# numz/ComfyUI-SeedVR2_VideoUpscaler

Measured on AMD Instinct MI355X. Metric: upscaled frames/sec (720p->4K, SeedVR2-3B), higher is better.
Workload: dtype bf16; 1 GPU; cfg3: SeedVR2-3B 32-frame 720p->4K clip (padded to 33 = 4n+1 for encode + DiT, 32 decoded), VAE tiled 1024/128; vae_tiled=True, parallelism=dp1, weights=random-init SeedVR2-3B + video_vae_v3 architecture (seeded)

## Files before the change

### comfyui-seedvr2_videoupscaler_amd/csrc/svr_conv_halo2.hip

```cpp
#include "svr_common.h"
#include "../../include/seedvr2_hip.h"
#include <type_traits>

namespace svr {

constexpr int CG_TX = 32, CG_HX = CG_TX + 2;
constexpr int CG_BUNIT = 128 * 64;
constexpr int CG_NB = 8;
constexpr int CG_D = 4;
static_assert(CG_D < CG_NB, "ring slot of unit k + D must not hold a unit still being read");

template <int TY, int MODE> struct cg_geom {
    static constexpr int MTW = MODE == 3 ? 8 : 4;
    static constexpr int NT = MODE == 3 ? 256 : TY * 32;
    static constexpr int HY = TY + 2;
    static constexpr int ROWS = CG_HX * HY;
    static constexpr int ACHUNKS = ROWS * 4;
    static constexpr int PIECES = (ACHUNKS + NT - 1) / NT;
    static constexpr int ABUF = MODE == 3 ? PIECES * NT * 16 : ROWS * 64;
    static constexpr int BOFF = 2 * ABUF;
    static constexpr int EP_ROWS = MODE ? 4 : 8;
    static constexpr int EP_BYTES = EP_ROWS * 32 * 528;
    static constexpr int THIN_PITCH = 272;
    static constexpr int MAIN = MODE == 2 ? TY * 32 * THIN_PITCH : (MODE == 1 || MODE == 3 ? BOFF : BOFF + CG_NB * CG_BUNIT);
    static constexpr int LDS = MAIN > EP_BYTES ? MAIN : EP_BYTES;
    static_assert(MODE == 3 || PIECES <= 7, "the next halo must have landed before interval 8");
};

template <int N> SVR_DEVICE void cg_wait_vmcnt() { asm volatile("s_waitcnt vmcnt(%0)" ::"n"(N) : "memory"); }
template <int OFF> SVR_DEVICE void cg_rd2(bf16x8 (&r)[2], unsigned a0) {
    asm volatile("ds_read_b128 %0, %2 offset:%3\n\tds_read_b128 %1, %2 offset:%4"
                 : "=&v"(r[0]), "=&v"(r[1]) : "v"(a0), "n"(OFF), "n"(OFF + 1024) : "memory");
}
SVR_DEVICE void cg_mm4(f32x4 (&c)[2][2], const bf16x8 (&w)[2], const bf16x8 (&r)[2]) {
    c[0][0] = __builtin_amdgcn_mfma_f32_16x16x32_bf16(w[0], r[0], c[0][0], 0, 0, 0);
    c[0][1] = __builtin_amdgcn_mfma_f32_16x16x32_bf16(w[1], r[0], c[0][1], 0, 0, 0);
    c[1][0] = __builtin_amdgcn_mfma_f32_16x16x32_bf16(w[0], r[1], c[1][0], 0, 0, 0);
    c[1][1] = __builtin_amdgcn_mfma_f32_16x16x32_bf16(w[1], r[1], c[1][1], 0, 0, 0);
}
SVR_DEVICE void cg_mm4_inplace(f32x4 (&c)[2][2], const bf16x8 (&w)[2], const bf16x8 (&r)[2]) {
    asm volatile("v_mfma_f32_16x16x32_bf16 %0, %1, %2, %0" : "+v"(c[0][0]) : "v"(w[0]), "v"(r[0]));
    asm volatile("v_mfma_f32_16x16x32_bf16 %0, %1, %2, %0" : "+v"(c[0][1]) : "v"(w[1]), "v"(r[0]));
    asm volatile("v_mfma_f32_16x16x32_bf16 %0, %1, %2, %0" : "+v"(c[1][0]) : "v"(w[0]), "v"(r[1]));
    asm volatile("v_mfma_f32_16x16x32_bf16 %0, %1, %2, %0" : "+v"(c[1][1]) : "v"(w[1]), "v"(r[1]));
}
template <int N> SVR_DEVICE void cg_wait_rows(bf16x8 (&a)[2]) {
    asm volatile("s_waitcnt lgkmcnt(%2)" : "+v"(a[0]), "+v"(a[1]) : "n"(N));
    __builtin_amdgcn_sched_barrier(0);
}
template <int N> SVR_DEVICE void cg_wait_rows(bf16x8 (&a)[2], bf16x8 (&b)[2]) {
    asm volatile("s_waitcnt lgkmcnt(%4)" : "+v"(a[0]), "+v"(a[1]), "+v"(b[0]), "+v"(b[1]) : "n"(N));
    __builtin_amdgcn_sched_barrier(0);
}
template <int N> SVR_DEVICE void cg_wait_rows(bf16x8 (&a)[2], bf16x8 (&b)[2], bf16x8 (&c)[2], bf16x8 (&d)[2], bf16x8 (&e)[2],
                                              bf16x8 (&f)[2], bf16x8 (&g)[2], bf16x8 (&h)[2]) {
    asm volatile("s_waitcnt lgkmcnt(%16)"
                 : "+v"(a[0]), "+v"(a[1]), "+v"(b[0]), "+v"(b[1]), "+v"(c[0]), "+v"(c[1]), "+v"(d[0]), "+v"(d[1]),
                   "+v"(e[0]), "+v"(e[1]), "+v"(f[0]), "+v"(f[1]), "+v"(g[0]), "+v"(g[1]), "+v"(h[0]), "+v"(h[1]) : "n"(N));
    __builtin_amdgcn_sched_barrier(0);
}
template <int N> SVR_DEVICE void cg_wait_w(bf16x8 (&w)[2][2]) {
    asm volatile("s_waitcnt vmcnt(%4)" : "+v"(w[0][0]), "+v"(w[0][1]), "+v"(w[1][0]), "+v"(w[1][1]) : "n"(N));
    __builtin_amdgcn_sched_barrier(0);
}

#ifdef SVR_ABLATIONS
__device__ unsigned long long g_conv_tl[4096][4];
__device__ unsigned long long g_conv_ep[4096][16];
#endif
template <int TY, int MODE, int DBG = 0>
__global__ __launch_bounds__((cg_geom<TY, MODE>::NT), (MODE == 3 ? 1 : 2)) void conv_halo2_kernel(const svr_gemm_args a, const int band_rows) {
#ifndef SVR_ABLATIONS
    static_assert(DBG == 0, "measurement variants (results invalid on purpose) exist only in -DSVR_ABLATIONS builds; the product library instantiates DBG = 0");
#endif
    typedef cg_geom<TY, MODE> G;
    constexpr bool WREG = MODE == 1 || MODE == 3, W8 = MODE == 3, THIN = MODE == 2;
    constexpr int CG_TY = TY, CG_ROWS = G::ROWS, CG_ABUF = G::ABUF, CG_ACHUNKS = G::ACHUNKS, CG_PIECES = G::PIECES,
                  CG_BOFF = G::BOFF, NT = G::NT;
    constexpr int MTW = G::MTW, NTW = 2;
    extern __shared__ __attribute__((aligned(16))) char smem[];

    const svr_conv_geom& g = a.conv;
    const int tid = threadIdx.x;
#ifdef SVR_ABLATIONS
    if constexpr ((DBG & 256) != 0) { if (tid == 0 && blockIdx.x < 4096) g_conv_tl[blockIdx.x][0] = __builtin_amdgcn_s_memtime(); }
#endif
    const int lane = tid & 63;
    const int wave = __builtin_amdgcn_readfirstlane(tid >> 6);
    const int grp = wave >> 2;
    const int wm = wave >> 1, wn = wave & 1;

    const int tiles_x = (g.W + CG_TX - 1) / CG_TX;
    const int tiles_y = (g.H + CG_TY - 1) / CG_TY;
    const int tiles_n = a.N / 128;
    int tl;
    {
        const int nwg = gridDim.x, bid = blockIdx.x;
        const int xcd = bid & 7, j = bid >> 3, q = nwg >> 3, r = nwg & 7;
        tl = (xcd < r ? xcd * (q + 1) : r * (q + 1) + (xcd - r) * q) + j;
    }
    const int tn = tl % tiles_n;
    int rr = tl / tiles_n;
    const int tx = rr % tiles_x; rr /= tiles_x;
    int ty, to;
    if (band_rows > 0 && band_rows < tiles_y) {
        const int per_band = band_rows * g.To;
        const int b = rr / per_band;
        const int rows_b = min(band_rows, tiles_y - b * band_rows);
        const int r2 = rr - b * per_band;
        to = r2 / rows_b;
        ty = b * band_rows + (r2 - to * rows_b);
    } else {
        ty = rr % tiles_y;
        to = rr / tiles_y;
    }
    const int y0 = ty * CG_TY, x0 = tx * CG_TX, n0 = tn * 128;

    const int cpk = THIN ? 1 : g.Cin / 32;
    const int nA = g.kt * cpk;
    const int P = nA * 9;
    const int64_t frame_bytes = (int64_t)g.H * g.W * g.Cin * 2;
    const int srow = tid >> 2, spos = tid & 3;
    const char* wbase = (const char*)a.W + (int64_t)(n0 + srow) * a.K * 2 + ((spos ^ ((srow >> 2) & 3)) * 16);
    uint32_t poff[CG_PIECES];
    uint32_t akeys = 0;
#pragma unroll
    for (int q = 0; q < CG_PIECES; ++q) {
        const int row = q * (NT / 4) + srow;
        const int hy = row / CG_HX, hx = row - hy * CG_HX;
        const int y = y0 - 1 + hy, x = x0 - 1 + hx;
        const bool ok = row < CG_ROWS && (unsigned)y < (unsigned)g.H && (unsigned)x < (unsigned)g.W;
        poff[q] = ok ? (uint32_t)(y * g.W + x) : 0xffffffffu;
        akeys |= (uint32_t)(spos ^ ((hx >> 2) & 3)) << (2 * q);
    }
    char* const wave_dst = smem + wave * 1024;

    auto frame_ptr = [&](int s) -> const char* {
        const int dt = s / cpk;
        const int c0 = (s - dt * cpk) * 32;
        int f = to + dt - g.pt;
        const char* basep = (const char*)a.A;
        if (f < 0) {
            if (g.halo != nullptr) { basep = (const char*)g.halo; f += g.halo_frames; }
            else f = 0;
        }
        return basep + (int64_t)f * frame_bytes + c0 * 2;
    };
    auto stage_a_piece = [&](auto qc, const char* fptr, int buf) {
        constexpr int Q = decltype(qc)::value;
        if (Q * NT + wave * 64 >= CG_ACHUNKS) return false;
        const int ck = (akeys >> (2 * Q)) & 3;
        const char* src = poff[Q] == 0xffffffffu ? (const char*)g.zeros
                                                 : fptr + ((int64_t)poff[Q] * g.Cin + ck * 8) * 2;
        if constexpr (!(DBG & 2))
            if (Q * NT + tid < CG_ACHUNKS) glds16(src, wave_dst + buf * CG_ABUF + Q * (NT * 16));
        return true;
    };
    auto stage_b = [&](int s, int tap, int slot) {
        const int dt = s / cpk;
        const int c0 = (s - dt * cpk) * 32;
        const int64_t koff = ((int64_t)(dt * 9 + tap) * g.Cin + c0) * 2;
        glds16(wbase + koff, wave_dst + CG_BOFF + slot * CG_BUNIT);
    };

    const int l15 = lane & 15, c4 = lane >> 4;
    int rd_a0[3], rd_b0;
#pragma unroll
    for (int dx = 0; dx < 3; ++dx)
        rd_a0[dx] = (wm * MTW * CG_HX + l15) * 64 + ((c4 ^ (((dx + l15) >> 2) & 3)) << 4);
    rd_b0 = CG_BOFF + (wn * 64 + l15) * 64 + ((c4 ^ ((l15 >> 2) & 3)) << 4);

    f32x4 acc[MTW][NTW][2][2];
#pragma unroll
    for (int y = 0; y < MTW; ++y)
#pragma unroll
        for (int z = 0; z < NTW; ++z)
#pragma unroll
            for (int e = 0; e < 16; ++e) acc[y][z][e >> 3][(e >> 2) & 1][e & 3] = 0.f;
    bf16x8 ar0[2], ar1[2], ar2[2], ar3[2], ar4[2], ar5[2], wf[NTW][2];
    bf16x8 ar6[2], ar7[2], ar8[2], ar9[2];

    auto reads = [&](auto jc, int s, int k) {
        constexpr int J = decltype(jc)::value;
        constexpr int DY = J % 3, DX = J / 3;
        int ra = rd_a0[DX] + (s & 1) * CG_ABUF;
        int rb = rd_b0 + (k & (CG_NB - 1)) * CG_BUNIT;
        asm volatile("" : "+v"(ra), "+v"(rb));
#pragma unroll
        for (int ks = 0; ks < 2; ++ks) {
            const char* pa = smem + ra + ks * 1024;
            const char* pb = smem + rb + ks * 1024;
            if constexpr (DY == 0) {
                ar0[ks] = *(const bf16x8*)(pa + (0 * CG_HX + DX) * 64);
                ar1[ks] = *(const bf16x8*)(pa + (1 * CG_HX + DX) * 64);
                ar2[ks] = *(const bf16x8*)(pa + (2 * CG_HX + DX) * 64);
                ar3[ks] = *(const bf16x8*)(pa + (3 * CG_HX + DX) * 64);
            } else if constexpr (DY == 1) {
                ar4[ks] = *(const bf16x8*)(pa + (4 * CG_HX + DX) * 64);
            } else {
                ar5[ks] = *(const bf16x8*)(pa + (5 * CG_HX + DX) * 64);
            }
#pragma unroll
            for (int nt = 0; nt < NTW; ++nt) wf[nt][ks] = *(const bf16x8*)(pb + nt * (32 * 64));
        }
    };
    auto mfma_core = [&](const bf16x8 (&r0)[2], const bf16x8 (&r1)[2], const bf16x8 (&r2)[2], const bf16x8 (&r3)[2]) {
        __builtin_amdgcn_s_setprio(1);
        cg_mm4(acc[0][0], wf[0], r0); cg_mm4(acc[0][1], wf[1], r0); cg_mm4(acc[1][0], wf[0], r1); cg_mm4(acc[1][1], wf[1], r1);
        cg_mm4(acc[2][0], wf[0], r2); cg_mm4(acc[2][1], wf[1], r2); cg_mm4(acc[3][0], wf[0], r3); cg_mm4(acc[3][1], wf[1], r3);
        __builtin_amdgcn_s_setprio(0);
    };
    auto mfmas = [&](auto jc) {
        constexpr int DY = decltype(jc)::value % 3;
        if constexpr (DY == 0) mfma_core(ar0, ar1, ar2, ar3);
        else if constexpr (DY == 1) mfma_core(ar1, ar2, ar3, ar4);
        else mfma_core(ar2, ar3, ar4, ar5);
    };

    if constexpr (THIN) {
        constexpr int TP = G::THIN_PITCH;
        static_assert(NT == 256, "one voxel per thread");
        const int taps = g.kt * 9;
        {
            const int y = y0 + (tid >> 5), x = x0 + (tid & 31);
            char* rowp = smem + tid * TP;
            const int64_t fpix = (int64_t)g.H * g.W;
            uint2 vv[32];
#pragma unroll
            for (int tap = 0; tap < 32; ++tap) {
                uint2 v = make_uint2(0u, 0u);
                if (tap < taps) {
                    const int dt = tap / 9, r = tap - dt * 9, dy = r / 3, dx = r - dy * 3;
                    const int ys = y + dy - 1, xs = x + dx - 1;
                    if ((unsigned)ys < (unsigned)g.H && (unsigned)xs < (unsigned)g.W) {
                        int f = to + dt - g.pt;
                        const char* basep = (const char*)a.A;
                        if (f < 0) {
                            if (g.halo != nullptr) { basep = (const char*)g.halo; f += g.halo_frames; }
                            else f = 0;
                        }
                        v = *(const uint2*)(basep + ((int64_t)f * fpix + (int64_t)ys * g.W + xs) * 8);
                    }
                }
                vv[tap] = v;
            }
#pragma unroll
            for (int tap = 0; tap < 32; tap += 2)
                *(uint4*)(rowp + tap * 8) = make_uint4(vv[tap].x, vv[tap].y, vv[tap + 1].x, vv[tap + 1].y);
        }
        __syncthreads();
        const int nks = (taps * 4 + 31) >> 5;
        const char* wrow0 = (const char*)a.W + ((int64_t)(n0 + wn * 64 + l15) * a.K + c4 * 8) * 2;
        const char* arow0 = smem + ((wm * MTW) * 32 + l15) * TP + c4 * 16;
#pragma unroll
        for (int ks = 0; ks < 4; ++ks) {
            if (ks < nks) {
                bf16x8 b[NTW][2];
#pragma unroll
                for (int q = 0; q < 2 * NTW; ++q) b[q >> 1][q & 1] = *(const bf16x8*)(wrow0 + (int64_t)(16 * q) * a.K * 2 + ks * 64);
#pragma unroll
                for (int mt = 0; mt < MTW; ++mt) {
                    bf16x8 av[2];
                    av[0] = *(const bf16x8*)(arow0 + mt * 32 * TP + ks * 64);
                    av[1] = *(const bf16x8*)(arow0 + (mt * 32 + 16) * TP + ks * 64);
                    cg_mm4(acc[mt][0], b[0], av);
                    cg_mm4(acc[mt][1], b[1], av);
                }
            }
        }
        __syncthreads();
    } else
    if constexpr (WREG) {
        const int64_t nstride = (int64_t)P * 2048;
        const char* wp0 = (const char*)a.W_frag + (int64_t)(n0 / 32 + wn * 2) * nstride;
        const char* wp1 = wp0 + nstride;
        const int voff = c4 * 512 + l15 * 16;
        bf16x8 w0[NTW][2], w1[NTW][2], w2[NTW][2];
        auto wload = [&](bf16x8 (&w)[NTW][2], int k) {
            if constexpr ((DBG & 32) != 0) k &= 3;
            auto uniform_ptr = [](const char* p) {
                const uint64_t u = (uint64_t)p;
                const uint32_t lo = __builtin_amdgcn_readfirstlane((uint32_t)u), hi = __builtin_amdgcn_readfirstlane((uint32_t)(u >> 32));
                return (const char*)(((uint64_t)hi << 32) | lo);
            };
            const char* p0 = uniform_ptr(wp0 + (int64_t)min(k, P - 1) * 2048);
            const char* p1 = uniform_ptr(wp1 + (int64_t)min(k, P - 1) * 2048);
            if constexpr ((DBG & 1) != 0 && W8) {
                if (k > 2) return;
            } else if constexpr (DBG & 1) {
                const bf16x8 z = {0, 0, 0, 0, 0, 0, 0, 0};
                w[0][0] = z; w[0][1] = z; w[1][0] = z; w[1][1] = z;
                return;
            }
            asm volatile("global_load_dwordx4 %0, %1, %2" : "=v"(w[0][0]) : "v"(voff), "s"(p0) : "memory");
            asm volatile("global_load_dwordx4 %0, %1, %2 offset:256" : "=v"(w[0][1]) : "v"(voff), "s"(p0) : "memory");
            asm volatile("global_load_dwordx4 %0, %1, %2" : "=v"(w[1][0]) : "v"(voff), "s"(p1) : "memory");
            asm volatile("global_load_dwordx4 %0, %1, %2 offset:256" : "=v"(w[1][1]) : "v"(voff), "s"(p1) : "memory");
        };
        auto reads_a = [&](auto jc, int s) {
            constexpr int J = decltype(jc)::value;
            constexpr int DY = J % 3, DX = J / 3;
            if constexpr ((DBG & 64) != 0) { if (s > 0) return; }
            int ra = rd_a0[DX] + (s & 1) * CG_ABUF;
            asm volatile("" : "+v"(ra));
#pragma unroll
            for (int ks = 0; ks < 2; ++ks) {
                const char* pa = smem + ra + ks * 1024;
                if constexpr (DY == 0) {
                    ar0[ks] = *(const bf16x8*)(pa + (0 * CG_HX + DX) * 64);
                    ar1[ks] = *(const bf16x8*)(pa + (1 * CG_HX + DX) * 64);
                    ar2[ks] = *(const bf16x8*)(pa + (2 * CG_HX + DX) * 64);
                    ar3[ks] = *(const bf16x8*)(pa + (3 * CG_HX + DX) * 64);
                } else if constexpr (DY == 1) {
                    ar4[ks] = *(const bf16x8*)(pa + (4 * CG_HX + DX) * 64);
                } else {
                    ar5[ks] = *(const bf16x8*)(pa + (5 * CG_HX + DX) * 64);
                }
            }
        };
        auto mfma_w = [&](const bf16x8 (&w)[NTW][2], const bf16x8 (&r0)[2], const bf16x8 (&r1)[2],
                          const bf16x8 (&r2)[2], const bf16x8 (&r3)[2]) {
            cg_mm4_inplace(acc[0][0], w[0], r0); cg_mm4_inplace(acc[0][1], w[1], r0);
            cg_mm4_inplace(acc[1][0], w[0], r1); cg_mm4_inplace(acc[1][1], w[1], r1);
            cg_mm4_inplace(acc[2][0], w[0], r2); cg_mm4_inplace(acc[2][1], w[1], r2);
            cg_mm4_inplace(acc[3][0], w[0], r3); cg_mm4_inplace(acc[3][1], w[1], r3);
        };
        if constexpr (W8) {
        const unsigned lds0 = (unsigned)(uintptr_t)(__attribute__((address_space(3))) char*)smem;
        unsigned fa[3];
#pragma unroll
        for (int dx = 0; dx < 3; ++dx) fa[dx] = lds0 + (unsigned)rd_a0[dx];
        auto stage_full = [&](auto qc, const char* fptr, int buf) {
            constexpr int Q = decltype(qc)::value;
            const int ck = (akeys >> (2 * Q)) & 3;
            const char* src = (poff[Q] == 0xffffffffu || fptr == nullptr) ? (const char*)g.zeros
                                                                          : fptr + ((int64_t)poff[Q] * g.Cin + ck * 8) * 2;
            glds16(src, wave_dst + buf * CG_ABUF + Q * (NT * 16));
        };
        static_assert(CG_PIECES == 10, "piece schedule below is written for ten pieces, two per interval 0..4");
        constexpr bool ABL_NO_DMA = (DBG & 16) != 0, ABL_NO_W = (DBG & 1) != 0, ABL_NO_RD = (DBG & 64) != 0;
#define SVR_RD(ROW, R, DXV, BUFOFF) do { if constexpr (!ABL_NO_RD) cg_rd2<((R) * CG_HX + (DXV)) * 64>(ROW, fa[DXV] + (BUFOFF)); } while (0)
#define SVR_MM8(W, RA, MA, RB, MB) \
        cg_mm4(acc[MA][0], W[0], RA); cg_mm4(acc[MA][1], W[1], RA); cg_mm4(acc[MB][0], W[0], RB); cg_mm4(acc[MB][1], W[1], RB)
        auto interval8 = [&](auto jc, int s, const char* fnext, bf16x8 (&wc)[NTW][2], bf16x8 (&wn_)[NTW][2]) {
            constexpr int J = decltype(jc)::value;
            constexpr int DY = J % 3, DX = J / 3;
            const int k = s * 9 + J;
            const unsigned cur = (unsigned)((s & 1) * CG_ABUF), nxt = (unsigned)(((s + 1) & 1) * CG_ABUF);
            constexpr int NPC[9] = {2, 2, 2, 2, 2, 0, 0, 0, 0};
            constexpr int NV = 4 + NPC[(J + 8) % 9] + NPC[(J + 7) % 9];
            if constexpr (DY == 0) {
                cg_wait_rows<0>(ar0, ar1, ar2, ar3, ar4, ar5, ar6, ar7);
                SVR_RD(ar8, 8, DX, cur);
                SVR_RD(ar9, 9, DX, cur);
            } else if constexpr (DY == 1 && J != 7) {
                cg_wait_rows<4>(ar8);
            } else if constexpr (DY == 2 && J != 8) {
                cg_wait_rows<4>(ar9);
            }
            if constexpr (!ABL_NO_DMA && !ABL_NO_W) cg_wait_w<NV>(wc);
            else if constexpr (ABL_NO_DMA && !ABL_NO_W) cg_wait_w<4>(wc);
            if constexpr (J == 7) SVR_RD(ar0, 0, 0, nxt);
            __builtin_amdgcn_sched_barrier(0);
            if constexpr (DY == 0) { SVR_MM8(wc, ar0, 0, ar1, 1); }
            else if constexpr (DY == 1) { SVR_MM8(wc, ar1, 0, ar2, 1); }
            else { SVR_MM8(wc, ar2, 0, ar3, 1); }
            __builtin_amdgcn_sched_barrier(0);
            if constexpr (DX < 2) {
                if constexpr (DY == 0) SVR_RD(ar0, 0, DX + 1, cur);
                else if constexpr (DY == 1) SVR_RD(ar1, 1, DX + 1, cur);
                else { SVR_RD(ar2, 2, DX + 1, cur); SVR_RD(ar3, 3, DX + 1, cur); }
            } else {
                if constexpr (DY == 1) SVR_RD(ar1, 1, 0, nxt);
                else if constexpr (DY == 2) { SVR_RD(ar2, 2, 0, nxt); SVR_RD(ar3, 3, 0, nxt); }
            }
            wload(wn_, k + 2);
            __builtin_amdgcn_sched_barrier(0);
            if constexpr (DY == 0) { SVR_MM8(wc, ar2, 2, ar3, 3); }
            else if constexpr (DY == 1) { SVR_MM8(wc, ar3, 2, ar4, 3); }
            else { SVR_MM8(wc, ar4, 2, ar5, 3); }
            __builtin_amdgcn_sched_barrier(0);
            if constexpr (DY == 2) {
                if constexpr (DX < 2) { SVR_RD(ar4, 4, DX + 1, cur); SVR_RD(ar5, 5, DX + 1, cur); }
                else { SVR_RD(ar4, 4, 0, nxt); SVR_RD(ar5, 5, 0, nxt); }
            }
            if constexpr (J < 5 && !ABL_NO_DMA) {
                stage_full(std::integral_constant<int, (J < 5 ? 2 * J : 0)>{}, fnext, (s + 1) & 1);
                stage_full(std::integral_constant<int, (J < 5 ? 2 * J + 1 : 0)>{}, fnext, (s + 1) & 1);
            }
            __builtin_amdgcn_sched_barrier(0);
            if constexpr (DY == 0) { SVR_MM8(wc, ar4, 4, ar5, 5); }
            else if constexpr (DY == 1) { SVR_MM8(wc, ar5, 4, ar6, 5); }
            else { SVR_MM8(wc, ar6, 4, ar7, 5); }
            __builtin_amdgcn_sched_barrier(0);
            if constexpr (DY == 2) {
                if constexpr (DX < 2) { SVR_RD(ar6, 6, DX + 1, cur); SVR_RD(ar7, 7, DX + 1, cur); }
                else { SVR_RD(ar6, 6, 0, nxt); SVR_RD(ar7, 7, 0, nxt); }
            }
            __builtin_amdgcn_sched_barrier(0);
            if constexpr (DY == 0) { SVR_MM8(wc, ar6, 6, ar7, 7); }
            else if constexpr (DY == 1) { SVR_MM8(wc, ar7, 6, ar8, 7); }
            else { SVR_MM8(wc, ar8, 6, ar9, 7); }
            __builtin_amdgcn_sched_barrier(0);
            if constexpr (J == 6) {
                cg_wait_rows<0>(ar8, ar9);
                if constexpr (!ABL_NO_DMA && !ABL_NO_W) cg_wait_vmcnt<8>();
                __builtin_amdgcn_s_barrier();
                __builtin_amdgcn_sched_barrier(0);
            }
        };
        {
            const char* f0 = frame_ptr(0);
            stage_full(std::integral_constant<int, 0>{}, f0, 0);
            stage_full(std::integral_constant<int, 1>{}, f0, 0);
            stage_full(std::integral_constant<int, 2>{}, f0, 0);
            stage_full(std::integral_constant<int, 3>{}, f0, 0);
            stage_full(std::integral_constant<int, 4>{}, f0, 0);
            stage_full(std::integral_constant<int, 5>{}, f0, 0);
            stage_full(std::integral_constant<int, 6>{}, f0, 0);
            stage_full(std::integral_constant<int, 7>{}, f0, 0);
            stage_full(std::integral_constant<int, 8>{}, f0, 0);
            stage_full(std::integral_constant<int, 9>{}, f0, 0);
            wload(w0, 0);
            wload(w1, 1);
            if constexpr (ABL_NO_W) wload(w2, 2);
            __builtin_amdgcn_sched_barrier(0);
#pragma unroll
            for (int y = 0; y < MTW; ++y)
#pragma unroll
                for (int z = 0; z < NTW; ++z)
                    asm volatile("" : "+a"(acc[y][z][0][0]), "+a"(acc[y][z][0][1]), "+a"(acc[y][z][1][0]), "+a"(acc[y][z][1][1]));
            cg_wait_vmcnt<0>();
            __builtin_amdgcn_s_barrier();
            __builtin_amdgcn_sched_barrier(0);
#define SVR_RD0(ROW, R) cg_rd2<((R) * CG_HX) * 64>(ROW, fa[0])
            SVR_RD0(ar0, 0); SVR_RD0(ar1, 1); SVR_RD0(ar2, 2); SVR_RD0(ar3, 3);
            SVR_RD0(ar4, 4); SVR_RD0(ar5, 5); SVR_RD0(ar6, 6); SVR_RD0(ar7, 7);
            if constexpr (ABL_NO_RD) { SVR_RD0(ar8, 8); SVR_RD0(ar9, 9); }
#undef SVR_RD0
        }
#ifdef SVR_ABLATIONS
        if constexpr ((DBG & 256) != 0) { if (tid == 0 && blockIdx.x < 4096) g_conv_tl[blockIdx.x][1] = __builtin_amdgcn_s_memtime(); }
#endif
        for (int s = 0; s < nA; ++s) {
            const char* fnext = s + 1 < nA ? frame_ptr((DBG & 128) ? 0 : s + 1) : nullptr;
            interval8(std::integral_constant<int, 0>{}, s, fnext, w0, w2);
            interval8(std::integral_constant<int, 1>{}, s, fnext, w1, w0);
            interval8(std::integral_constant<int, 2>{}, s, fnext, w2, w1);
            interval8(std::integral_constant<int, 3>{}, s, fnext, w0, w2);
            interval8(std::integral_constant<int, 4>{}, s, fnext, w1, w0);
            interval8(std::integral_constant<int, 5>{}, s, fnext, w2, w1);
            interval8(std::integral_constant<int, 6>{}, s, fnext, w0, w2);
            interval8(std::integral_constant<int, 7>{}, s, fnext, w1, w0);
            interval8(std::integral_constant<int, 8>{}, s, fnext, w2, w1);
        }
        cg_wait_vmcnt<0>();
        asm volatile("s_waitcnt lgkmcnt(0)" ::: "memory");
        __builtin_amdgcn_sched_barrier(0);
#undef SVR_RD
#undef SVR_MM8
        } else {
        bool a_prev3 = false;
        auto interval3 = [&](auto jc, int s, const char* fnext, const bf16x8 (&wc)[NTW][2], bf16x8 (&wn_)[NTW][2]) {
            constexpr int J = decltype(jc)::value;
            constexpr int DY = J % 3;
            const int k = s * 9 + J;
            bool a_issued = false;
            if constexpr (J < CG_PIECES && !(DBG & 16)) {
                if (s + 1 < nA) a_issued = stage_a_piece(std::integral_constant<int, (J < CG_PIECES ? J : 0)>{}, fnext, (s + 1) & 1);
            }
            wload(wn_, k + 2);
            reads_a(jc, s);
            {
                const int n = 8 + (a_issued ? 1 : 0) + (a_prev3 ? 1 : 0);
                if (n == 10) cg_wait_vmcnt<10>(); else if (n == 9) cg_wait_vmcnt<9>(); else cg_wait_vmcnt<8>();
            }
            a_prev3 = a_issued;
            asm volatile("s_waitcnt lgkmcnt(0)" ::: "memory");
            __builtin_amdgcn_sched_barrier(0);
            if (grp == 0) __builtin_amdgcn_s_setprio(2); else __builtin_amdgcn_s_setprio(1);
            if constexpr (DY == 0) mfma_w(wc, ar0, ar1, ar2, ar3);
            else if constexpr (DY == 1) mfma_w(wc, ar1, ar2, ar3, ar4);
            else mfma_w(wc, ar2, ar3, ar4, ar5);
            __builtin_amdgcn_s_setprio(0);
            __builtin_amdgcn_sched_barrier(0);
            if constexpr (J == 8) {
                if (s + 1 < nA) cg_wait_vmcnt<8>(); else cg_wait_vmcnt<0>();
                if constexpr (!(DBG & 8)) __builtin_amdgcn_s_barrier();
                __builtin_amdgcn_sched_barrier(0);
            }
        };
        {
            const char* f0 = frame_ptr(0);
            stage_a_piece(std::integral_constant<int, 0>{}, f0, 0);
            stage_a_piece(std::integral_constant<int, 1>{}, f0, 0);
            stage_a_piece(std::integral_constant<int, 2>{}, f0, 0);
            stage_a_piece(std::integral_constant<int, 3>{}, f0, 0);
            stage_a_piece(std::integral_constant<int, 4>{}, f0, 0);
            if constexpr (CG_PIECES > 5) stage_a_piece(std::integral_constant<int, (CG_PIECES > 5 ? 5 : 0)>{}, f0, 0);
            static_assert(CG_PIECES <= 6, "prologue stages at most six pieces");
            if constexpr ((DBG & 16) != 0) {
                stage_a_piece(std::integral_constant<int, 0>{}, f0, 1);
                stage_a_piece(std::integral_constant<int, 1>{}, f0, 1);
                stage_a_piece(std::integral_constant<int, 2>{}, f0, 1);
                stage_a_piece(std::integral_constant<int, 3>{}, f0, 1);
                stage_a_piece(std::integral_constant<int, 4>{}, f0, 1);
                if constexpr (CG_PIECES > 5) stage_a_piece(std::integral_constant<int, (CG_PIECES > 5 ? 5 : 0)>{}, f0, 1);
            }
            wload(w0, 0);
            wload(w1, 1);
            cg_wait_vmcnt<0>();
            __builtin_amdgcn_s_barrier();
            __builtin_amdgcn_sched_barrier(0);
        }
#ifdef SVR_ABLATIONS
        if constexpr ((DBG & 256) != 0) { if (tid == 0 && blockIdx.x < 4096) g_conv_tl[blockIdx.x][1] = __builtin_amdgcn_s_memtime(); }
#endif
        for (int s = 0; s < nA; ++s) {
            const char* fnext = frame_ptr((DBG & 128) ? 0 : min(s + 1, nA - 1));
            interval3(std::integral_constant<int, 0>{}, s, fnext, w0, w2);
            interval3(std::integral_constant<int, 1>{}, s, fnext, w1, w0);
            interval3(std::integral_constant<int, 2>{}, s, fnext, w2, w1);
            interval3(std::integral_constant<int, 3>{}, s, fnext, w0, w2);
            interval3(std::integral_constant<int, 4>{}, s, fnext, w1, w0);
            interval3(std::integral_constant<int, 5>{}, s, fnext, w2, w1);
            interval3(std::integral_constant<int, 6>{}, s, fnext, w0, w2);
            interval3(std::integral_constant<int, 7>{}, s, fnext, w1, w0);
            interval3(std::integral_constant<int, 8>{}, s, fnext, w2, w1);
        }
        asm volatile("s_nop 7\n\ts_nop 7" ::: "memory");
        }
    } else {
    {
        const char* f0 = frame_ptr(0);
        stage_a_piece(std::integral_constant<int, 0>{}, f0, 0);
        stage_a_piece(std::integral_constant<int, 1>{}, f0, 0);
        stage_a_piece(std::integral_constant<int, 2>{}, f0, 0);
        stage_a_piece(std::integral_constant<int, 3>{}, f0, 0);
        stage_a_piece(std::integral_constant<int, 4>{}, f0, 0);
#pragma unroll
        for (int u = 0; u < CG_D; ++u) stage_b(0, (u % 3) * 3 + u / 3, u);
        cg_wait_vmcnt<0>();
        __builtin_amdgcn_s_barrier();
    }
    if (grp == 0) {
        reads(std::integral_constant<int, 0>{}, 0, 0);
        asm volatile("s_waitcnt lgkmcnt(0)" ::: "memory");
    }
    __builtin_amdgcn_sched_barrier(0);

    bool a_prev = false;
    auto interval = [&](auto jc, int s, const char* fnext) {
        constexpr int J = decltype(jc)::value;
        const int k = s * 9 + J;
        if (grp == 0) {
            mfmas(jc);
            if constexpr (J + 1 < 9) reads(std::integral_constant<int, (J + 1) % 9>{}, s, k + 1);
            else if (s + 1 < nA) reads(std::integral_constant<int, 0>{}, s + 1, k + 1);
        } else {
            reads(jc, s, k);
        }
        bool a_issued = false;
        if constexpr (J < CG_PIECES) {
            if (s + 1 < nA) a_issued = stage_a_piece(std::integral_constant<int, (J < CG_PIECES ? J : 0)>{}, fnext, (s + 1) & 1);
        }
        const bool b_issued = k + CG_D < P;
        if (b_issued) {
            constexpr int JU = (J + CG_D) % 9;
            stage_b(s + (J + CG_D) / 9, (JU % 3) * 3 + JU / 3, (k + CG_D) & (CG_NB - 1));
        }
        static_assert(CG_D == 4, "counts below are written for a prefetch distance of 4");
        if (b_issued) {
            const int n = 2 + (a_issued ? 1 : 0) + (a_prev ? 1 : 0);
            if (n == 4) cg_wait_vmcnt<4>(); else if (n == 3) cg_wait_vmcnt<3>(); else cg_wait_vmcnt<2>();
        } else {
            cg_wait_vmcnt<0>();
        }
        a_prev = a_issued;
        asm volatile("s_waitcnt lgkmcnt(0)" ::: "memory");
        __builtin_amdgcn_sched_barrier(0);
        if (grp == 1) mfmas(jc);
        __builtin_amdgcn_sched_barrier(0);
        __builtin_amdgcn_s_barrier();
        __builtin_amdgcn_sched_barrier(0);
    };

    for (int s = 0; s < nA; ++s) {
        const char* fnext = frame_ptr(min(s + 1, nA - 1));
        interval(std::integral_constant<int, 0>{}, s, fnext);
        interval(std::integral_constant<int, 1>{}, s, fnext);
        interval(std::integral_constant<int, 2>{}, s, fnext);
        interval(std::integral_constant<int, 3>{}, s, fnext);
        interval(std::integral_constant<int, 4>{}, s, fnext);
        interval(std::integral_constant<int, 5>{}, s, fnext);
        interval(std::integral_constant<int, 6>{}, s, fnext);
        interval(std::integral_constant<int, 7>{}, s, fnext);
        interval(std::integral_constant<int, 8>{}, s, fnext);
    }

    }

#ifdef SVR_ABLATIONS
    if constexpr ((DBG & 256) != 0) { if (tid == 0 && blockIdx.x < 4096) g_conv_tl[blockIdx.x][2] = __builtin_amdgcn_s_memtime(); }
#endif
    constexpr int EP_PITCH = 528;
    f32x4 bias_lo = {0.f, 0.f, 0.f, 0.f}, bias_hi = {0.f, 0.f, 0.f, 0.f};
    if (a.bias) {
        bias_lo = *(const f32x4*)(a.bias + n0 + (tid & 15) * 8);
        bias_hi = *(const f32x4*)(a.bias + n0 + (tid & 15) * 8 + 4);
    }
#ifdef SVR_ABLATIONS
#define SVR_EP_STAMP(i) if constexpr ((DBG & 256) != 0) { if (tid == 0 && blockIdx.x < 4096) g_conv_ep[blockIdx.x][i] = __builtin_amdgcn_s_memtime(); }
#else
#define SVR_EP_STAMP(i)
#endif
    SVR_EP_STAMP(0)
    const bool resid_gate = a.epilogue == SVR_EPI_RESID_GATE;
    double gs0 = 0.0, gq0 = 0.0, gs1 = 0.0, gq1 = 0.0;
    constexpr int EP_ROWS = G::EP_ROWS;
    constexpr int NPASS = MTW / 2;
    static_assert(TY / EP_ROWS == NPASS && EP_ROWS * 32 * 16 == 8 * NT, "MTW / 2 passes, eight store iterations each");
    auto ep_body = [&](auto fc) {
        constexpr int F = decltype(fc)::value;
        constexpr bool RT = F < 0, F_RESID = !RT && (F & 1), F_GN = !RT && (F & 2);
        const bool with_resid = RT ? (resid_gate && a.resid != nullptr) : F_RESID;
        const int ko = RT ? a.out_f32 : ((F & 4) != 0 ? SVR_STORE_H16 : SVR_STORE_BF16);
        const int kr = RT ? a.resid_f32 : ((F & 8) != 0 ? SVR_STORE_H16 : SVR_STORE_BF16);
        const bool o32 = ko == SVR_STORE_FP32, r32 = kr == SVR_STORE_FP32;
        const bool with_gn = RT ? a.gn_partial != nullptr : F_GN;
        constexpr bool PRE = W8 && !RT && F_RESID;
        uint4 rpre[2][8];
        auto resid_prefetch = [&](auto pc, uint4 (&dst)[8]) {
            constexpr int P = decltype(pc)::value;
            const int n_ = n0 + (tid & 15) * 8;
#pragma unroll
            for (int q = 0; q < 8; ++q) {
                const int vox = (q * NT + tid) >> 4;
                const int r = vox >> 5;
                const int y = y0 + (r >> 1) * MTW + 2 * P + (r & 1), x = x0 + (vox & 31);
                const int64_t m_ = ((int64_t)to * g.H + min(y, g.H - 1)) * g.W + min(x, g.W - 1);
                dst[q] = *(const uint4*)((const bf16_t*)a.resid + m_ * a.ldr + n_);
            }
        };
        if constexpr (PRE) resid_prefetch(std::integral_constant<int, 0>{}, rpre[0]);
#pragma unroll
        for (int pass = 0; pass < NPASS; ++pass) {
#pragma unroll
            for (int j = 0; j < 2; ++j) {
#pragma unroll
                for (int vh = 0; vh < 2; ++vh) {
                    char* row = smem + ((wm * 2 + j) * 32 + vh * 16 + l15) * EP_PITCH;
#pragma unroll
                    for (int nt = 0; nt < NTW; ++nt)
#pragma unroll
                        for (int ch = 0; ch < 2; ++ch)
                            *(f32x4*)(row + (wn * 64 + nt * 32 + ch * 16 + c4 * 4) * 4) = acc[2 * pass + j][nt][vh][ch];
                }
            }
            SVR_EP_STAMP(1 + 3 * pass)
            if constexpr ((DBG & 512) != 0) __syncthreads(); else lds_barrier();
            SVR_EP_STAMP(2 + 3 * pass)
            if constexpr (PRE) {
                if (pass + 1 < NPASS) {
                    if (pass == 0) resid_prefetch(std::integral_constant<int, 1>{}, rpre[1]);
                    else if (pass == 1) resid_prefetch(std::integral_constant<int, 2>{}, rpre[0]);
                    else if (pass == 2) resid_prefetch(std::integral_constant<int, 3>{}, rpre[1]);
                }
            }
            const int n = n0 + (tid & 15) * 8;
#pragma unroll
            for (int half = 0; half < 2; ++half) {
            f32x4 lo[4], hi_[4];
            uint4 rr8[4];
            f32x4 rf0[4], rf1[4];
            int64_t mrow[4];
            bool ok[4];
#pragma unroll
            for (int it = 0; it < 4; ++it) {
                const int vox = ((half * 4 + it) * NT + tid) >> 4;
                const int r = vox >> 5;
                const int y = y0 + (r >> 1) * MTW + 2 * pass + (r & 1), x = x0 + (vox & 31);
                ok[it] = y < g.H && x < g.W;
                if constexpr ((DBG & 4) != 0) ok[it] = false;
                mrow[it] = ((int64_t)to * g.H + min(y, g.H - 1)) * g.W + min(x, g.W - 1);
                lo[it] = *(const f32x4*)(smem + vox * EP_PITCH + (tid & 15) * 32);
                hi_[it] = *(const f32x4*)(smem + vox * EP_PITCH + (tid & 15) * 32 + 16);
            }
            if (with_resid) {
                if constexpr (RT) {
                    if (!r32) {
#pragma unroll
                        for (int it = 0; it < 4; ++it) rr8[it] = *(const uint4*)((const bf16_t*)a.resid + mrow[it] * a.ldr + n);
                    }
                } else if (r32) {
#pragma unroll
                    for (int it = 0; it < 4; ++it) {
                        const float* rp = (const float*)a.resid + mrow[it] * a.ldr + n;
                        rf0[it] = *(const f32x4*)rp;
                        rf1[it] = *(const f32x4*)(rp + 4);
                    }
                } else {
                    if constexpr (PRE) {
#pragma unroll
                        for (int it = 0; it < 4; ++it) rr8[it] = rpre[pass & 1][half * 4 + it];
                    } else {
#pragma unroll
                        for (int it = 0; it < 4; ++it) rr8[it] = *(const uint4*)((const bf16_t*)a.resid + mrow[it] * a.ldr + n);
                    }
                }
            }
#pragma unroll
            for (int it = 0; it < 4; ++it) {
                float f[8] = {lo[it][0] + bias_lo[0], lo[it][1] + bias_lo[1], lo[it][2] + bias_lo[2], lo[it][3] + bias_lo[3],
                              hi_[it][0] + bias_hi[0], hi_[it][1] + bias_hi[1], hi_[it][2] + bias_hi[2], hi_[it][3] + bias_hi[3]};
                if constexpr (RT) {
                    if (a.epilogue == SVR_EPI_BIAS_SILU) {
#pragma unroll
                        for (int e = 0; e < 8; ++e) f[e] = silu(f[e]);
                    }
                    if (resid_gate && a.gate) {
#pragma unroll
                        for (int e = 0; e < 8; ++e) f[e] *= a.gate[n + e];
                    }
                }
                if (with_resid) {
                    float r8[8];
                    if (r32) {
                        if constexpr (RT) {
                            const float* rp = (const float*)a.resid + mrow[it] * a.ldr + n;
                            rf0[0] = *(const f32x4*)rp;
                            rf1[0] = *(const f32x4*)(rp + 4);
                        }
#pragma unroll
                        for (int e = 0; e < 4; ++e) { r8[e] = rf0[RT ? 0 : it][e]; r8[4 + e] = rf1[RT ? 0 : it][e]; }
                    } else if (kr == SVR_STORE_H16) {
                        unpack8h(rr8[it], r8);
                    } else {
                        unpack8(rr8[it], r8);
                    }
#pragma unroll
                    for (int e = 0; e < 8; ++e) f[e] += r8[e];
                }
                if (o32) {
                    if (ok[it]) {
                        float* cp = (float*)a.C + mrow[it] * a.ldc + n;
                        *(float4*)cp = make_float4(f[0], f[1], f[2], f[3]);
                        *(float4*)(cp + 4) = make_float4(f[4], f[5], f[6], f[7]);
                        if (with_gn) {
                            gn_accumulate4(gs0, gq0, f[0], f[1], f[2], f[3]);
                            gn_accumulate4(gs1, gq1, f[4], f[5], f[6], f[7]);
                        }
                    }
                } else {
                    const uint4 pk = ko == SVR_STORE_H16 ? pack8h(f) : pack8(f);
                    if (ok[it]) *(uint4*)((bf16_t*)a.C + mrow[it] * a.ldc + n) = pk;
                    if (with_gn && ok[it]) {
                        float r[8];
                        if (ko == SVR_STORE_H16) unpack8h(pk, r); else unpack8(pk, r);
                        gn_accumulate4(gs0, gq0, r[0], r[1], r[2], r[3]);
                        gn_accumulate4(gs1, gq1, r[4], r[5], r[6], r[7]);
                    }
                }
            }
            }
            SVR_EP_STAMP(3 + 3 * pass)
            if (pass + 1 < NPASS) { if constexpr ((DBG & 512) != 0) __syncthreads(); else lds_barrier(); }
        }
    };
    const bool wr = resid_gate && a.resid != nullptr;
    if (a.epilogue != SVR_EPI_BIAS_SILU && a.gate == nullptr && a.out_f32 != SVR_STORE_FP32 && !(wr && a.resid_f32 == SVR_STORE_FP32) &&
        (DBG == 0 || (!a.out_f32 && !a.resid_f32))) {
        const int F = (wr ? 1 : 0) | (a.gn_partial != nullptr ? 2 : 0) | (a.out_f32 == SVR_STORE_H16 ? 4 : 0) |
                      (wr && a.resid_f32 == SVR_STORE_H16 ? 8 : 0);
        switch (F) {
#define SVR_EP_CASE(v) case v: ep_body(std::integral_constant<int, v>{}); break;
            SVR_EP_CASE(0) SVR_EP_CASE(1) SVR_EP_CASE(2) SVR_EP_CASE(3)
            default:
                if constexpr (DBG == 0) switch (F) {
                    SVR_EP_CASE(4) SVR_EP_CASE(5) SVR_EP_CASE(6) SVR_EP_CASE(7) SVR_EP_CASE(9) SVR_EP_CASE(11) SVR_EP_CASE(13) SVR_EP_CASE(15)
                    default: break;
                }
                break;
#undef SVR_EP_CASE
        }
    } else {
        ep_body(std::integral_constant<int, -1>{});
    }
    if (a.gn_partial) {
        __syncthreads();
        static_assert(NT * 32 + 32 * 16 <= G::LDS, "statistics staging fits the kernel's LDS");
        double4* red = (double4*)smem;
        double2* qsum = (double2*)(smem + NT * 32);
        red[tid] = make_double4(gs0, gq0, gs1, gq1);
        __syncthreads();
        if (tid < 32) {
            const int c = tid >> 1, h = tid & 1;
            double s = 0.0, q = 0.0;
            for (int j = 0; j < NT / 16; ++j) {
                const double4 v = red[(j << 4) | c];
                s += h ? v.z : v.x;
                q += h ? v.w : v.y;
            }
            qsum[tid] = make_double2(s, q);
        }
        __syncthreads();
        const int qpg = (a.N / a.gn_groups) >> 2;
        if (tid < 32 / qpg) {
            double s = 0.0, q = 0.0;
            for (int i = 0; i < qpg; ++i) { s += qsum[tid * qpg + i].x; q += qsum[tid * qpg + i].y; }
            const int blk = ty * tiles_x + tx, nblk = tiles_y * tiles_x;
            ((double2*)a.gn_partial)[((int64_t)to * nblk + blk) * a.gn_groups + (n0 >> 2) / qpg + tid] = make_double2(s, q);
        }
    }
#ifdef SVR_ABLATIONS
    if constexpr ((DBG & 256) != 0) {
        if (tid == 0 && blockIdx.x < 4096) g_conv_tl[blockIdx.x][3] = __builtin_amdgcn_s_memtime();
    }
#endif
}

int g_conv_band = 1;
int g_conv_rows = 8;
int g_conv_lds_dbg = 0;
static bool conv_halo2_wreg(const svr_gemm_args& a) { return a.W_frag != nullptr && g_conv_impl == 0; }

template <int TY, int MODE, int DBG = 0> static int launch_conv_halo2_t(const svr_gemm_args& a, hipStream_t s) {
    typedef cg_geom<TY, MODE> G;
    const svr_conv_geom& g = a.conv;
    const int tiles = g.To * ((g.H + TY - 1) / TY) * ((g.W + CG_TX - 1) / CG_TX) * (a.N / 128);
    static uint64_t lds_attr_done = 0;
    {
        const int e = set_max_dynamic_lds((const void*)conv_halo2_kernel<TY, MODE, DBG>, 160 * 1024, lds_attr_done);
        if (e != 0) return e;
    }
    hipLaunchKernelGGL((conv_halo2_kernel<TY, MODE, DBG>), dim3(tiles), dim3(G::NT), g_conv_lds_dbg > G::LDS ? g_conv_lds_dbg : G::LDS, s, a,
                       g_conv_band);
    return (int)hipGetLastError();
}

static int launch_conv_halo2(const svr_gemm_args& a, hipStream_t s) {
#ifdef SVR_ABLATIONS
#include "measure/svr_conv_halo2_measure_1.inc"
#endif
    if (conv_halo2_wreg(a)) return g_conv_rows == 8 ? launch_conv_halo2_t<16, 3>(a, s) : launch_conv_halo2_t<8, 1>(a, s);
    return launch_conv_halo2_t<16, 0>(a, s);
}

static bool conv_halo2_out_layout(const svr_gemm_args& a) {
    return (a.ldc % 8) == 0 && ((uintptr_t)a.C % 16) == 0 && (!a.resid || ((a.ldr % 8) == 0 && ((uintptr_t)a.resid % 16) == 0)) &&
           (!a.bias || ((uintptr_t)a.bias % 16) == 0);
}
static bool conv_thin_geometry(const svr_gemm_args& a) {
    const svr_conv_geom& g = a.conv;
    return g.enabled && g.Cin == 4 && g.kh == 3 && g.kw == 3 && g.sh == 1 && g.sw == 1 && g.st == 1 &&
           g.ph == 1 && g.pw == 1 && g.Ho == g.H && g.Wo == g.W && g.kt >= 1 && g.kt <= 3 && a.K == 128 &&
           g.To == g.T + g.pt - g.kt + 1 && !a.ps.enabled && a.epilogue != SVR_EPI_SWIGLU && a.epilogue != SVR_EPI_BIAS_GELU &&
           (a.N % 128) == 0;
}
static bool conv_thin_eligible(const svr_gemm_args& a) { return conv_thin_geometry(a) && conv_halo2_out_layout(a); }
static int launch_conv_thin(const svr_gemm_args& a, hipStream_t s) { return launch_conv_halo2_t<8, 2>(a, s); }

static int conv_gn_blocks(const svr_gemm_args& a) {
    if (a.gn_groups > 0 && conv_sub_eligible(a)) return conv_sub_gn_blocks(a);
    if (conv_thin_eligible(a) && a.gn_groups > 0) {
        const int cpg = a.N / a.gn_groups;
        if (cpg < 4 || (cpg & 3) || a.N % a.gn_groups || 128 % cpg) return 0;
        return ((a.conv.H + 7) / 8) * ((a.conv.W + CG_TX - 1) / CG_TX);
    }
    if ((g_conv_impl != 0 && g_conv_impl != 3) || !conv_halo_eligible(a) || (a.N % 128) != 0 || a.conv.Cin % 32 != 0) return 0;
    const int cpg = a.gn_groups > 0 ? a.N / a.gn_groups : 0;
    if (cpg < 4 || (cpg & 3) || a.N % a.gn_groups || 128 % cpg) return 0;
    const int ty = conv_halo2_wreg(a) && g_conv_rows != 8 ? 8 : 16;
    return ((a.conv.H + ty - 1) / ty) * ((a.conv.W + CG_TX - 1) / CG_TX);
}

static bool conv_halo_eligible(const svr_gemm_args& a) {
    const svr_conv_geom& g = a.conv;
    return g.enabled && g.kh == 3 && g.kw == 3 && g.sh == 1 && g.sw == 1 && g.st == 1 && g.ph == 1 && g.pw == 1 &&
           g.Ho == g.H && g.Wo == g.W && g.Cin % 64 == 0 && g.kt >= 1 && g.kt <= 3 &&
           g.To == g.T + g.pt - g.kt + 1 && !a.ps.enabled && !a.phase.enabled && a.epilogue != SVR_EPI_SWIGLU &&
           (a.N <= 32 || ((a.N % 128) == 0 && conv_halo2_out_layout(a))) &&
           (int64_t)g.H * g.W * g.Cin * 2 < (int64_t)1 << 32;
}

static bool conv_halo2_eligible(const svr_gemm_args& a) {
    return conv_halo_eligible(a) && (a.N % 128) == 0 && a.conv.Cin % 32 == 0 && a.epilogue != SVR_EPI_BIAS_GELU;
}

__global__ __launch_bounds__(256) void conv_pack_frag_kernel(const bf16_t* __restrict__ W, uint4* __restrict__ out, int N, int K,
                                                             int kt, int Cin) {
    const int cpk = Cin / 32, P = kt * cpk * 9;
    const int64_t idx = (int64_t)blockIdx.x * 256 + threadIdx.x;
    if (idx >= (int64_t)(N / 32) * P * 128) return;
    const int lane = (int)(idx & 63), ks = (int)((idx >> 6) & 1);
    const int kk = (int)((idx >> 7) % P), n32 = (int)((idx >> 7) / P);
    const int s = kk / 9, J = kk - s * 9;
    const int dt = s / cpk, cs = s - dt * cpk, dy = J % 3, dx = J / 3;
    const int n = n32 * 32 + (lane & 31), c = cs * 32 + ks * 16 + (lane >> 5) * 8;
    out[idx] = *(const uint4*)(W + (int64_t)n * K + ((dt * 9 + dy * 3 + dx) * Cin + c));
}

}
```

Baseline: 3.657 frames/s.

## Interleave LDS reads, weight loads and DMA between individual MFMAs in conv interval

Rewrites the W8 register-weight conv inner interval so each of the 16 MFMA units is followed by one scheduled side op: an LDS row read, one of the four weight global loads, or half of an activation-piece DMA. Before, these ran as grouped blocks between MFMA batches. Weight pointers now advance incrementally instead of being recomputed with readfirstlane and min clamps, and the next-frame pointer comes from running counters instead of a division. The aim is a smoother instruction issue mix that hides memory latency behind matrix ops, at the cost of many more sched barriers that may constrain the compiler.

Result: faster. 3.748 frames/s, median of 6 (+2.5%).

```diff
diff --git a/comfyui-seedvr2_videoupscaler_amd/csrc/svr_conv_halo2.hip b/comfyui-seedvr2_videoupscaler_amd/csrc/svr_conv_halo2.hip
--- a/comfyui-seedvr2_videoupscaler_amd/csrc/svr_conv_halo2.hip
+++ b/comfyui-seedvr2_videoupscaler_amd/csrc/svr_conv_halo2.hip
@@ -135,9 +135,8 @@
     }
     char* const wave_dst = smem + wave * 1024;
 
-    auto frame_ptr = [&](int s) -> const char* {
-        const int dt = s / cpk;
-        const int c0 = (s - dt * cpk) * 32;
+    auto frame_ptr_at = [&](int dt, int c) -> const char* {
+        const int c0 = c * 32;
         int f = to + dt - g.pt;
         const char* basep = (const char*)a.A;
         if (f < 0) {
@@ -145,6 +144,10 @@
             else f = 0;
         }
         return basep + (int64_t)f * frame_bytes + c0 * 2;
+    };
+    auto frame_ptr = [&](int s) -> const char* {
+        const int dt = s / cpk;
+        return frame_ptr_at(dt, s - dt * cpk);
     };
     auto stage_a_piece = [&](auto qc, const char* fptr, int buf) {
         constexpr int Q = decltype(qc)::value;
@@ -285,9 +288,7 @@
             };
             const char* p0 = uniform_ptr(wp0 + (int64_t)min(k, P - 1) * 2048);
             const char* p1 = uniform_ptr(wp1 + (int64_t)min(k, P - 1) * 2048);
-            if constexpr ((DBG & 1) != 0 && W8) {
-                if (k > 2) return;
-            } else if constexpr (DBG & 1) {
+            if constexpr (DBG & 1) {
                 const bf16x8 z = {0, 0, 0, 0, 0, 0, 0, 0};
                 w[0][0] = z; w[0][1] = z; w[1][0] = z; w[1][1] = z;
                 return;
@@ -330,78 +331,104 @@
         unsigned fa[3];
 #pragma unroll
         for (int dx = 0; dx < 3; ++dx) fa[dx] = lds0 + (unsigned)rd_a0[dx];
-        auto stage_full = [&](auto qc, const char* fptr, int buf) {
+        auto piece_src = [&](auto qc, const char* fptr) -> const char* {
             constexpr int Q = decltype(qc)::value;
             const int ck = (akeys >> (2 * Q)) & 3;
             const char* src = (poff[Q] == 0xffffffffu || fptr == nullptr) ? (const char*)g.zeros
                                                                           : fptr + ((int64_t)poff[Q] * g.Cin + ck * 8) * 2;
+            asm volatile("" : "+v"(src));
+            return src;
+        };
+        auto piece_dma = [&](auto qc, const char* src, int buf) {
+            constexpr int Q = decltype(qc)::value;
             glds16(src, wave_dst + buf * CG_ABUF + Q * (NT * 16));
         };
+        auto stage_full = [&](auto qc, const char* fptr, int buf) { piece_dma(qc, piece_src(qc, fptr), buf); };
         static_assert(CG_PIECES == 10, "piece schedule below is written for ten pieces, two per interval 0..4");
         constexpr bool ABL_NO_DMA = (DBG & 16) != 0, ABL_NO_W = (DBG & 1) != 0, ABL_NO_RD = (DBG & 64) != 0;
-#define SVR_RD(ROW, R, DXV, BUFOFF) do { if constexpr (!ABL_NO_RD) cg_rd2<((R) * CG_HX + (DXV)) * 64>(ROW, fa[DXV] + (BUFOFF)); } while (0)
-#define SVR_MM8(W, RA, MA, RB, MB) \
-        cg_mm4(acc[MA][0], W[0], RA); cg_mm4(acc[MA][1], W[1], RA); cg_mm4(acc[MB][0], W[0], RB); cg_mm4(acc[MB][1], W[1], RB)
-        auto interval8 = [&](auto jc, int s, const char* fnext, bf16x8 (&wc)[NTW][2], bf16x8 (&wn_)[NTW][2]) {
+        int voff0 = voff, voff1 = voff + (int)nstride;
+        const char* wq = wp0;
+        auto wl = [&](auto ic, bf16x8 (&w)[NTW][2]) {
+            constexpr int I = decltype(ic)::value;
+            const int o0 = voff0, o1 = voff1;
+            const char* const q = wq;
+            if constexpr (I == 0) asm volatile("global_load_dwordx4 %0, %1, %2" : "=v"(w[0][0]) : "v"(o0), "s"(q) : "memory");
+            else if constexpr (I == 1) asm volatile("global_load_dwordx4 %0, %1, %2 offset:256" : "=v"(w[0][1]) : "v"(o0), "s"(q) : "memory");
+            else if constexpr (I == 2) asm volatile("global_load_dwordx4 %0, %1, %2" : "=v"(w[1][0]) : "v"(o1), "s"(q) : "memory");
+            else asm volatile("global_load_dwordx4 %0, %1, %2 offset:256" : "=v"(w[1][1]) : "v"(o1), "s"(q) : "memory");
+        };
+        auto wload_all = [&](bf16x8 (&w)[NTW][2]) {
+            wl(std::integral_constant<int, 0>{}, w); wl(std::integral_constant<int, 1>{}, w);
+            wl(std::integral_constant<int, 2>{}, w); wl(std::integral_constant<int, 3>{}, w);
+            wq += 2048;
+        };
+        auto rowref = [&](auto rc) -> bf16x8 (&)[2] {
+            constexpr int R = decltype(rc)::value;
+            static_assert(R >= 0 && R <= 9, "ten halo rows per column shift");
+            if constexpr (R == 0) return ar0; else if constexpr (R == 1) return ar1; else if constexpr (R == 2) return ar2;
+            else if constexpr (R == 3) return ar3; else if constexpr (R == 4) return ar4; else if constexpr (R == 5) return ar5;
+            else if constexpr (R == 6) return ar6; else if constexpr (R == 7) return ar7; else if constexpr (R == 8) return ar8;
+            else return ar9;
+        };
+        auto interval8 = [&](auto jc, int s, const char* fnext, int wadv, bf16x8 (&wc)[NTW][2], bf16x8 (&wn_)[NTW][2]) {
             constexpr int J = decltype(jc)::value;
             constexpr int DY = J % 3, DX = J / 3;
-            const int k = s * 9 + J;
+            constexpr int NDX = DX < 2 ? DX + 1 : 0;
             const unsigned cur = (unsigned)((s & 1) * CG_ABUF), nxt = (unsigned)(((s + 1) & 1) * CG_ABUF);
+            const unsigned nbuf = DX < 2 ? cur : nxt;
             constexpr int NPC[9] = {2, 2, 2, 2, 2, 0, 0, 0, 0};
             constexpr int NV = 4 + NPC[(J + 8) % 9] + NPC[(J + 7) % 9];
-            if constexpr (DY == 0) {
-                cg_wait_rows<0>(ar0, ar1, ar2, ar3, ar4, ar5, ar6, ar7);
-                SVR_RD(ar8, 8, DX, cur);
-                SVR_RD(ar9, 9, DX, cur);
-            } else if constexpr (DY == 1 && J != 7) {
-                cg_wait_rows<4>(ar8);
-            } else if constexpr (DY == 2 && J != 8) {
-                cg_wait_rows<4>(ar9);
-            }
+            if constexpr (DY == 0) cg_wait_rows<0>(ar0, ar1, ar2, ar3, ar4, ar5, ar6, ar7);
+            else if constexpr (DY == 1 && J != 7) cg_wait_rows<4>(ar8);
+            else if constexpr (DY == 2 && J != 8) cg_wait_rows<4>(ar9);
             if constexpr (!ABL_NO_DMA && !ABL_NO_W) cg_wait_w<NV>(wc);
             else if constexpr (ABL_NO_DMA && !ABL_NO_W) cg_wait_w<4>(wc);
-            if constexpr (J == 7) SVR_RD(ar0, 0, 0, nxt);
             __builtin_amdgcn_sched_barrier(0);
-            if constexpr (DY == 0) { SVR_MM8(wc, ar0, 0, ar1, 1); }
-            else if constexpr (DY == 1) { SVR_MM8(wc, ar1, 0, ar2, 1); }
-            else { SVR_MM8(wc, ar2, 0, ar3, 1); }
-            __builtin_amdgcn_sched_barrier(0);
-            if constexpr (DX < 2) {
-                if constexpr (DY == 0) SVR_RD(ar0, 0, DX + 1, cur);
-                else if constexpr (DY == 1) SVR_RD(ar1, 1, DX + 1, cur);
-                else { SVR_RD(ar2, 2, DX + 1, cur); SVR_RD(ar3, 3, DX + 1, cur); }
-            } else {
-                if constexpr (DY == 1) SVR_RD(ar1, 1, 0, nxt);
-                else if constexpr (DY == 2) { SVR_RD(ar2, 2, 0, nxt); SVR_RD(ar3, 3, 0, nxt); }
-            }
-            wload(wn_, k + 2);
-            __builtin_amdgcn_sched_barrier(0);
-            if constexpr (DY == 0) { SVR_MM8(wc, ar2, 2, ar3, 3); }
-            else if constexpr (DY == 1) { SVR_MM8(wc, ar3, 2, ar4, 3); }
-            else { SVR_MM8(wc, ar4, 2, ar5, 3); }
-            __builtin_amdgcn_sched_barrier(0);
-            if constexpr (DY == 2) {
-                if constexpr (DX < 2) { SVR_RD(ar4, 4, DX + 1, cur); SVR_RD(ar5, 5, DX + 1, cur); }
-                else { SVR_RD(ar4, 4, 0, nxt); SVR_RD(ar5, 5, 0, nxt); }
-            }
-            if constexpr (J < 5 && !ABL_NO_DMA) {
-                stage_full(std::integral_constant<int, (J < 5 ? 2 * J : 0)>{}, fnext, (s + 1) & 1);
-                stage_full(std::integral_constant<int, (J < 5 ? 2 * J + 1 : 0)>{}, fnext, (s + 1) & 1);
-            }
-            __builtin_amdgcn_sched_barrier(0);
-            if constexpr (DY == 0) { SVR_MM8(wc, ar4, 4, ar5, 5); }
-            else if constexpr (DY == 1) { SVR_MM8(wc, ar5, 4, ar6, 5); }
-            else { SVR_MM8(wc, ar6, 4, ar7, 5); }
-            __builtin_amdgcn_sched_barrier(0);
-            if constexpr (DY == 2) {
-                if constexpr (DX < 2) { SVR_RD(ar6, 6, DX + 1, cur); SVR_RD(ar7, 7, DX + 1, cur); }
-                else { SVR_RD(ar6, 6, 0, nxt); SVR_RD(ar7, 7, 0, nxt); }
-            }
-            __builtin_amdgcn_sched_barrier(0);
-            if constexpr (DY == 0) { SVR_MM8(wc, ar6, 6, ar7, 7); }
-            else if constexpr (DY == 1) { SVR_MM8(wc, ar7, 6, ar8, 7); }
-            else { SVR_MM8(wc, ar8, 6, ar9, 7); }
-            __builtin_amdgcn_sched_barrier(0);
+            constexpr bool PIECES_HERE = J < 5 && !ABL_NO_DMA;
+            constexpr int QA = J < 5 ? 2 * J : 0, QB = J < 5 ? 2 * J + 1 : 0;
+            const char* srca = nullptr;
+            const char* srcb = nullptr;
+            auto rd = [&](auto rc, auto dxc, unsigned bufoff) {
+                constexpr int R = decltype(rc)::value, DXV = decltype(dxc)::value;
+                if constexpr (!ABL_NO_RD) cg_rd2<(R * CG_HX + DXV) * 64>(rowref(rc), fa[DXV] + bufoff);
+            };
+            auto rdn = [&](auto rc) { rd(rc, std::integral_constant<int, NDX>{}, nbuf); };
+            auto side = [&](auto uc) {
+                constexpr int U = decltype(uc)::value;
+                constexpr int WL0 = DY == 2 ? 2 : 3;
+                if constexpr (!ABL_NO_W && U >= WL0 && U <= WL0 + 6 && (U - WL0) % 2 == 0) {
+                    wl(std::integral_constant<int, (U - WL0) / 2>{}, wn_);
+                    if constexpr (U == WL0 + 6) {
+                        if constexpr (J == 6 || J == 7) wq += wadv; else wq += 2048;
+                    }
+                }
+                if constexpr (DY == 0) {
+                    if constexpr (U == 0) rd(std::integral_constant<int, 8>{}, std::integral_constant<int, DX>{}, cur);
+                    else if constexpr (U == 1) rd(std::integral_constant<int, 9>{}, std::integral_constant<int, DX>{}, cur);
+                    else if constexpr (U == 2 && DX < 2) rdn(std::integral_constant<int, 0>{});
+                } else if constexpr (DY == 1) {
+                    if constexpr (U == 0 && J == 7) rdn(std::integral_constant<int, 0>{});
+                    else if constexpr (U == 1) rdn(std::integral_constant<int, 1>{});
+                } else {
+                    if constexpr (U <= 11 && U % 2 == 1) rdn(std::integral_constant<int, 2 + U / 2>{});
+                }
+                if constexpr (PIECES_HERE) {
+                    if constexpr (U == 10) srca = piece_src(std::integral_constant<int, QA>{}, fnext);
+                    else if constexpr (U == 12) piece_dma(std::integral_constant<int, QA>{}, srca, (s + 1) & 1);
+                    else if constexpr (U == 13) srcb = piece_src(std::integral_constant<int, QB>{}, fnext);
+                    else if constexpr (U == 14) piece_dma(std::integral_constant<int, QB>{}, srcb, (s + 1) & 1);
+                }
+                __builtin_amdgcn_sched_barrier(0);
+            };
+            auto unit = [&](auto uc) {
+                constexpr int U = decltype(uc)::value;
+                cg_mm4(acc[U / 2][U & 1], wc[U & 1], rowref(std::integral_constant<int, U / 2 + DY>{}));
+                __builtin_amdgcn_sched_barrier(0);
+            };
+#define SVR_US(U) unit(std::integral_constant<int, U>{}); side(std::integral_constant<int, U>{})
+            SVR_US(0); SVR_US(1); SVR_US(2); SVR_US(3); SVR_US(4); SVR_US(5); SVR_US(6); SVR_US(7);
+            SVR_US(8); SVR_US(9); SVR_US(10); SVR_US(11); SVR_US(12); SVR_US(13); SVR_US(14); SVR_US(15);
+#undef SVR_US
             if constexpr (J == 6) {
                 cg_wait_rows<0>(ar8, ar9);
                 if constexpr (!ABL_NO_DMA && !ABL_NO_W) cg_wait_vmcnt<8>();
@@ -421,9 +448,9 @@
             stage_full(std::integral_constant<int, 7>{}, f0, 0);
             stage_full(std::integral_constant<int, 8>{}, f0, 0);
             stage_full(std::integral_constant<int, 9>{}, f0, 0);
-            wload(w0, 0);
-            wload(w1, 1);
-            if constexpr (ABL_NO_W) wload(w2, 2);
+            wload_all(w0);
+            wload_all(w1);
+            if constexpr (ABL_NO_W) wload_all(w2);
             __builtin_amdgcn_sched_barrier(0);
 #pragma unroll
             for (int y = 0; y < MTW; ++y)
@@ -442,23 +469,25 @@
 #ifdef SVR_ABLATIONS
         if constexpr ((DBG & 256) != 0) { if (tid == 0 && blockIdx.x < 4096) g_conv_tl[blockIdx.x][1] = __builtin_amdgcn_s_memtime(); }
 #endif
+        int ndt = 0, nc = 0;
         for (int s = 0; s < nA; ++s) {
-            const char* fnext = s + 1 < nA ? frame_ptr((DBG & 128) ? 0 : s + 1) : nullptr;
-            interval8(std::integral_constant<int, 0>{}, s, fnext, w0, w2);
-            interval8(std::integral_constant<int, 1>{}, s, fnext, w1, w0);
-            interval8(std::integral_constant<int, 2>{}, s, fnext, w2, w1);
-            interval8(std::integral_constant<int, 3>{}, s, fnext, w0, w2);
-            interval8(std::integral_constant<int, 4>{}, s, fnext, w1, w0);
-            interval8(std::integral_constant<int, 5>{}, s, fnext, w2, w1);
-            interval8(std::integral_constant<int, 6>{}, s, fnext, w0, w2);
-            interval8(std::integral_constant<int, 7>{}, s, fnext, w1, w0);
-            interval8(std::integral_constant<int, 8>{}, s, fnext, w2, w1);
+            if (++nc == cpk) { nc = 0; ++ndt; }
+            const bool more = s + 1 < nA;
+            const char* fnext = more ? frame_ptr_at(ndt, nc) : nullptr;
+            const int wadv = more ? 2048 : 0;
+            interval8(std::integral_constant<int, 0>{}, s, fnext, wadv, w0, w2);
+            interval8(std::integral_constant<int, 1>{}, s, fnext, wadv, w1, w0);
+            interval8(std::integral_constant<int, 2>{}, s, fnext, wadv, w2, w1);
+            interval8(std::integral_constant<int, 3>{}, s, fnext, wadv, w0, w2);
+            interval8(std::integral_constant<int, 4>{}, s, fnext, wadv, w1, w0);
+            interval8(std::integral_constant<int, 5>{}, s, fnext, wadv, w2, w1);
+            interval8(std::integral_constant<int, 6>{}, s, fnext, wadv, w0, w2);
+            interval8(std::integral_constant<int, 7>{}, s, fnext, wadv, w1, w0);
+            interval8(std::integral_constant<int, 8>{}, s, fnext, wadv, w2, w1);
         }
         cg_wait_vmcnt<0>();
         asm volatile("s_waitcnt lgkmcnt(0)" ::: "memory");
         __builtin_amdgcn_sched_barrier(0);
-#undef SVR_RD
-#undef SVR_MM8
         } else {
         bool a_prev3 = false;
         auto interval3 = [&](auto jc, int s, const char* fnext, const bf16x8 (&wc)[NTW][2], bf16x8 (&wn_)[NTW][2]) {
```
